# kije/gpu_raytracer

Measured on AMD Instinct MI355X. Metric: Mrays/s, higher is better.
Workload: dtype f32

## Files before the change

### gpu_raytracer_amd/csrc/device_common.h

```cpp
#ifndef RT_DEVICE_COMMON_H
#define RT_DEVICE_COMMON_H

#include <hip/hip_runtime.h>
#include <stdint.h>

#include "device_layout.h"

namespace rtdev {

#define RT_MIN_RAY_DISTANCE 0.00001f
#define RT_F32_MAX 3.402823466e+38f
#define RT_PI 3.14159265358979323846f
#define WAVE 64


struct V3 {
    float x, y, z;
};
__device__ __forceinline__ V3 v3(float x, float y, float z) { return V3{x, y, z}; }
__device__ __forceinline__ V3 ld3(const float* p) { return V3{p[0], p[1], p[2]}; }
__device__ __forceinline__ V3 operator+(V3 a, V3 b) { return v3(a.x + b.x, a.y + b.y, a.z + b.z); }
__device__ __forceinline__ V3 operator-(V3 a, V3 b) { return v3(a.x - b.x, a.y - b.y, a.z - b.z); }
__device__ __forceinline__ V3 operator*(V3 a, V3 b) { return v3(a.x * b.x, a.y * b.y, a.z * b.z); }
__device__ __forceinline__ V3 operator*(V3 a, float s) { return v3(a.x * s, a.y * s, a.z * s); }
// ... 128 lines not shown
}
__device__ __forceinline__ uint32_t ray_octant(const FilterRay& f) {
    return (f.inv.x < 0.0f ? 1u : 0u) | (f.inv.y < 0.0f ? 2u : 0u) | (f.inv.z < 0.0f ? 4u : 0u);
}
__device__ __forceinline__ uint32_t first_slot(uint32_t m, uint32_t oct) {
    uint32_t p = m & 0xFFu;
    if (oct & 1u) p = ((p & 0x55u) << 1) | ((p >> 1) & 0x55u);
    if (oct & 2u) p = ((p & 0x33u) << 2) | ((p >> 2) & 0x33u);
    if (oct & 4u) p = ((p & 0x0Fu) << 4) | (p >> 4);
    return ((uint32_t)__ffs((int)p) - 1u) ^ oct;
}

typedef float f32x2 __attribute__((ext_vector_type(2)));

template <bool COUNT>
__device__ __forceinline__ uint32_t visit_node8(const uint4* __restrict__ nodes, uint32_t idx, const FilterRay& fr, float closest_t, Counts& cnt,
                                                uint32_t& child_base, uint32_t& tri_base, uint32_t& imask, uint32_t& lmask) {
    const uint4* n = nodes + (size_t)idx * 5;
    const uint4 w0 = n[0], w1 = n[1], w2 = n[2], w3 = n[3], w4 = n[4];
    uint32_t w1x = w1.x, w1y = w1.y, w1z = w1.z;
    asm volatile("" : "+v"(w1x), "+v"(w1y), "+v"(w1z));
    if (COUNT) cnt.nodes++;
    const float ax = ldexpf(fr.inv.x, (int)(int8_t)(w0.w & 0xFFu)), ay = ldexpf(fr.inv.y, (int)(int8_t)((w0.w >> 8) & 0xFFu)),
                az = ldexpf(fr.inv.z, (int)(int8_t)((w0.w >> 16) & 0xFFu));
    const float dox = __uint_as_float(w0.x) - fr.o.x, doy = __uint_as_float(w0.y) - fr.o.y, doz = __uint_as_float(w0.z) - fr.o.z;
    const float bx = dox * fr.inv.x, by = doy * fr.inv.y, bz = doz * fr.inv.z;
    const float ex = fmaf(255.0f, fabsf(ax), fabsf(bx)) * RT_FILTER_SLACK;
    const float ey = fmaf(255.0f, fabsf(ay), fabsf(by)) * RT_FILTER_SLACK;
    const float ez = fmaf(255.0f, fabsf(az), fabsf(bz)) * RT_FILTER_SLACK;
    const f32x2 pm = {-1.0f, 1.0f};
    const f32x2 bx2 = __builtin_elementwise_fma((f32x2){ex, ex}, pm, (f32x2){bx, bx});
    const f32x2 by2 = __builtin_elementwise_fma((f32x2){ey, ey}, pm, (f32x2){by, by});
    const f32x2 bz2 = __builtin_elementwise_fma((f32x2){ez, ez}, pm, (f32x2){bz, bz});
    const f32x2 ax2 = {ax, ax}, ay2 = {ay, ay}, az2 = {az, az};
    const bool px = fr.inv.x >= 0.0f, py = fr.inv.y >= 0.0f, pz = fr.inv.z >= 0.0f;
    const uint32_t nxw[2] = {px ? w2.x : w3.z, px ? w2.y : w3.w}, fxw[2] = {px ? w3.z : w2.x, px ? w3.w : w2.y};
    const uint32_t nyw[2] = {py ? w2.z : w4.x, py ? w2.w : w4.y}, fyw[2] = {py ? w4.x : w2.z, py ? w4.y : w2.w};
    const uint32_t nzw[2] = {pz ? w3.x : w4.z, pz ? w3.y : w4.w}, fzw[2] = {pz ? w4.z : w3.x, pz ? w4.w : w3.y};
    const float limit = closest_t * 1.0000153f;
    uint32_t miss = 0;
#pragma unroll
    for (int h = 1; h >= 0; h--) {
#pragma unroll
        for (int i = 3; i >= 0; i--) {
            const f32x2 qx = {(float)((nxw[h] >> (8 * i)) & 0xFFu), (float)((fxw[h] >> (8 * i)) & 0xFFu)};
            const f32x2 qy = {(float)((nyw[h] >> (8 * i)) & 0xFFu), (float)((fyw[h] >> (8 * i)) & 0xFFu)};
            const f32x2 qz = {(float)((nzw[h] >> (8 * i)) & 0xFFu), (float)((fzw[h] >> (8 * i)) & 0xFFu)};
            const f32x2 tx = __builtin_elementwise_fma(qx, ax2, bx2);
            const f32x2 ty = __builtin_elementwise_fma(qy, ay2, by2);
            const f32x2 tz = __builtin_elementwise_fma(qz, az2, bz2);
            const float tmin = fmaxf(fmaxf(tx.x, ty.x), fmaxf(tz.x, 0.0f));
            const float tmax = fminf(fminf(tx.y, ty.y), fminf(tz.y, limit));
            miss = __builtin_amdgcn_alignbit(miss, __float_as_uint(tmax - tmin), 31);
        }
    }
    child_base = w1x;
    tri_base = w1y;
    lmask = w1z & 0xFFu;
    imask = w0.w >> 24;
    return ~miss & (imask | lmask);
}

template <bool COUNT, bool ANY_HIT>
__device__ __forceinline__ void traverse(const DevScene& sc, V3 o, V3 d, uint2* __restrict__ stack, Hit& hit, Counts& cnt, float tmin) {
    if (sc.n_nodes == 0) return;
    const FilterRay fr = make_filter_ray(o, d);
    const uint32_t oct = ray_octant(fr);
    const uint4* __restrict__ nodes = reinterpret_cast<const uint4*>(sc.nodes);
    uint32_t g_base = 0, g_bits = 1u | (1u << 8);
    int sp = 0;
    for (;;) {
        if ((g_bits & 0xFFu) == 0u) {
            if (sp == 0) break;
            sp--;
            const uint2 e = stack[sp * WAVE];
            g_base = e.x;
            g_bits = e.y;
        }
        const uint32_t i = first_slot(g_bits, oct);
        g_bits ^= 1u << i;
        const uint32_t node = g_base + (uint32_t)__popc(__builtin_amdgcn_ubfe(g_bits, 8u, i));
        if (g_bits & 0xFFu) {
            stack[sp * WAVE] = make_uint2(g_base, g_bits);
            sp++;
        }
        uint32_t cb, tb, im, lm;
        const uint32_t hm = visit_node8<COUNT>(nodes, node, fr, hit.t, cnt, cb, tb, im, lm);
        uint32_t t = hm & lm;
        while (t) {
            const uint32_t sl = first_slot(t, oct);
            t ^= 1u << sl;
            const uint32_t first = tb + RT_DEV_LEAF_STRIDE * (uint32_t)__popc(lm & ((1u << sl) - 1u));
            if (test_leaf<COUNT, ANY_HIT>(sc.tris, RT_DEV_LEAF_FLAG | first, o, d, hit, cnt, tmin)) return;
        }
        g_base = cb;
        g_bits = (hm & im) | (im << 8);
    }
}

template <bool COUNT>
__device__ __forceinline__ Hit find_closest(const DevScene& sc, V3 o, V3 d, uint2* stack, Counts& cnt) {
    Hit hit;
    hit.t = RT_F32_MAX;
    hit.prim = RT_PRIM_MISS;
    hit.slot = 0;
    test_spheres(sc, o, d, hit, RT_MIN_RAY_DISTANCE);
    traverse<COUNT, false>(sc, o, d, stack, hit, cnt, RT_MIN_RAY_DISTANCE);
    return hit;
}

template <bool COUNT>
__device__ __forceinline__ bool occluded(const DevScene& sc, V3 o, V3 d, float tmin, float tmax, uint2* stack, Counts& cnt) {
    Hit h;
    h.t = tmax;
    h.prim = RT_PRIM_MISS;
    h.slot = 0;
    test_spheres(sc, o, d, h, tmin);
    if (h.prim != RT_PRIM_MISS) return true;
    traverse<COUNT, true>(sc, o, d, stack, h, cnt, tmin);
    return h.prim != RT_PRIM_MISS;
}

__device__ __forceinline__ V3 evaluate_brdf(const DevMaterial& m, float intensity) {
    V3 albedo = ld3(m.albedo);
    V3 diffuse = albedo / RT_PI;
    float is_metallic = (m.metallic > 0.5f) ? 1.0f : 0.0f;
    V3 metallic_contrib = albedo * intensity * 0.5f;
    V3 dielectric_contrib = diffuse * intensity;
    return metallic_contrib * is_metallic + dielectric_contrib * (1.0f - is_metallic);
}

__device__ __forceinline__ V3 light_contribution(const DevLight& L, const DevMaterial& m, V3 point, V3 normal, V3& to_light_dir,
                                                 float& to_light_dist) {
    V3 dir_light_dir = ld3(L.neg_ndir);
    float dir_intensity = fmaxf(dot(normal, dir_light_dir), 0.0f) * L.intensity;
    V3 to_light = ld3(L.position) - point;
    float distance = length(to_light);
    V3 pld = normalize(to_light);
    float att = f16_round_trip(1.0f / (1.0f + distance * distance * 0.01f));
    float point_intensity = fmaxf(dot(normal, pld), 0.0f) * L.intensity * att;
    float spot_factor = fmaxf(dot(dir_light_dir, pld), 0.0f);
    float spot_intensity = point_intensity * spot_factor;
    float is_dir = (L.light_type == 0) ? 1.0f : 0.0f;
    float is_point = (L.light_type == 1) ? 1.0f : 0.0f;
    float is_spot = (L.light_type == 2) ? 1.0f : 0.0f;
    float final_i = dir_intensity * is_dir + point_intensity * is_point + spot_intensity * is_spot;
    V3 brdf = evaluate_brdf(m, final_i);
    float valid = (final_i > 0.0f) ? 1.0f : 0.0f;
    to_light_dir = (L.light_type == 0) ? dir_light_dir : pld;
    to_light_dist = (L.light_type == 0) ? RT_F32_MAX : distance;
    return brdf * ld3(L.color) * valid;
}

__device__ __forceinline__ V3 calculate_lighting(const DevScene& sc, const DevMaterial& m, V3 point, V3 normal) {
    V3 total = v3(0.0f, 0.0f, 0.0f);
    total = total + ld3(m.albedo) * 0.1f;
    for (uint32_t li = 0; li < sc.n_lights; li++) {
        V3 sd;
        float st;
        total = total + light_contribution(sc.lights[li], m, point, normal, sd, st);
    }
    return total + ld3(m.emission);
}

__device__ __forceinline__ void surface_at(const DevScene& sc, bool sphere, uint32_t slot, V3 point, V3& normal, uint32_t& material_id) {
    if (sphere) {
        const DevSphere& s = sc.spheres[slot];
        normal = normalize(point - ld3(s.center));
        material_id = s.material_id;
    } else {
        const float4* p = reinterpret_cast<const float4*>(sc.tris + slot);
        float4 q0 = p[0], q1 = p[1], q2 = p[2];
        asm volatile("" : "+v"(q0.w), "+v"(q1.x), "+v"(q1.y), "+v"(q1.z), "+v"(q1.w), "+v"(q2.x), "+v"(q2.y));
        V3 e1 = v3(q0.w, q1.x, q1.y);
        V3 e2 = v3(q1.z, q1.w, q2.x);
        normal = normalize(cross(e1, e2));
        material_id = __float_as_uint(q2.y);
    }
}
__device__ __forceinline__ void hit_geometry(const DevScene& sc, const Hit& hit, V3 o, V3 d, V3& point, V3& normal, uint32_t& material_id) {
    point = o + d * hit.t;
    surface_at(sc, (hit.prim & RT_PRIM_SPHERE_FLAG) != 0, hit.slot, point, normal, material_id);
}

__device__ __forceinline__ V3 transmission_mix(const DevMaterial& m, V3 lighting, float tf) {
    float disp_r = ((m.ior + -0.018f) - 1.0f) / (m.ior - 1.0f);
    float disp_g = ((m.ior + 0.0f) - 1.0f) / (m.ior - 1.0f);
    float disp_b = ((m.ior + 0.035f) - 1.0f) / (m.ior - 1.0f);
    float keep = 1.0f - tf;
    return v3(lighting.x * keep + (0.2f * disp_r) * tf, lighting.y * keep + (0.2f * disp_g) * tf,
              lighting.z * keep + (0.3f * disp_b) * tf);
}

__device__ __forceinline__ V3 shade_hit(const DevScene& sc, const Hit& hit, V3 o, V3 d) {
    V3 point, normal;
    uint32_t material_id;
    hit_geometry(sc, hit, o, d, point, normal, material_id);
    if (material_id >= sc.n_materials) return v3(1.0f, 0.0f, 1.0f);
    const DevMaterial m = sc.materials[material_id];
    V3 lighting = calculate_lighting(sc, m, point, normal);
    float tf = fminf(fmaxf(m.transmission, 0.0f), 1.0f);
    if (tf > 0.0f) return transmission_mix(m, lighting, tf);
    return lighting;
}

__device__ __forceinline__ uint32_t unorm8(float v) {
    if (!(v > 0.0f)) return 0u;
    if (v >= 1.0f) return 255u;
    return (uint32_t)floorf(v * 255.0f + 0.5f);
}

struct PixelCoord {
    uint32_t x, y;
    bool valid;
};
__device__ __forceinline__ PixelCoord block_pixel_at(const DevFrame& fr, uint32_t block, uint32_t lane) {
    uint32_t ox, oy, tw, th, blk;
    const uint32_t bpt_x = (fr.tile_size + 7u) >> 3;
    if (fr.single_tile) {
        ox = fr.tile_off_x; oy = fr.tile_off_y; tw = fr.tile_w; th = fr.tile_h;
        blk = block;
    } else {
        const uint32_t bpt = bpt_x * bpt_x;
        uint32_t k = block / bpt;
        blk = block - k * bpt;
        uint32_t tile = fr.tile_first + k * fr.tile_stride;
        uint32_t ty = tile / fr.tiles_x, tx = tile - ty * fr.tiles_x;
        ox = tx * fr.tile_size; oy = ty * fr.tile_size;
        tw = min(fr.tile_size, fr.width - ox);
        th = min(fr.tile_size, fr.height - oy);
    }
    uint32_t by = blk / bpt_x, bx = blk - by * bpt_x;
    uint32_t idx = bx * 8u + (lane & 7u), idy = by * 8u + (lane >> 3);
    PixelCoord pc;
    pc.x = ox + idx;
    pc.y = oy + idy;
    pc.valid = idx < tw && idy < th && pc.x < fr.width && pc.y < fr.height;
    return pc;
}
__device__ __forceinline__ PixelCoord block_pixel(const DevFrame& fr) { return block_pixel_at(fr, blockIdx.x, threadIdx.x); }

struct SimpleRng {
    uint32_t seed;
    __device__ __forceinline__ uint32_t next_u32() {
        seed = seed * 1664525u + 1013904223u;
        return seed;
    }
    __device__ __forceinline__ float next_f32() { return (float)(next_u32() >> 8) / 16777216.0f; }
};

__device__ __forceinline__ SimpleRng rng_for(uint32_t pixel_seed, uint32_t sample) {
    uint32_t h = pixel_seed + sample * 0x9E3779B9u;
    h ^= h >> 16;
    h *= 0x7FEB352Du;
    h ^= h >> 15;
    h *= 0x846CA68Bu;
    h ^= h >> 16;
    return SimpleRng{h};
}

__device__ __forceinline__ V3 run_sum_start(const DevFrame& fr, const DevTargets& tg, size_t pix) {
    if (!tg.run_sum || fr.sample_base == 0) return v3(0.0f, 0.0f, 0.0f);
    const float4 a = reinterpret_cast<const float4*>(tg.run_sum)[pix];
    return v3(a.x, a.y, a.z);
}
__device__ __forceinline__ void run_sum_keep(const DevTargets& tg, size_t pix, V3 sum) {
    if (tg.run_sum) reinterpret_cast<float4*>(tg.run_sum)[pix] = make_float4(sum.x, sum.y, sum.z, 0.0f);
}

__device__ __forceinline__ void sincos_2pi(float u, float& s_out, float& c_out) {
    float f4 = u * 4.0f;
    float qf = floorf(f4);
    int q = (int)qf;
    float x = (f4 - qf) * 1.57079632679489661923f;
    float x2 = x * x;
    float sp = __builtin_fmaf(x2, -2.50521083854417187751e-8f, 2.75573192239858906526e-6f);
    sp = __builtin_fmaf(x2, sp, -1.98412698412698412698e-4f);
    sp = __builtin_fmaf(x2, sp, 8.33333333333333333333e-3f);
    sp = __builtin_fmaf(x2, sp, -1.66666666666666666667e-1f);
    sp = __builtin_fmaf(x2, sp, 1.0f);
    float sn = x * sp;
    float cp = __builtin_fmaf(x2, 2.08767569878680989792e-9f, -2.75573192239858906526e-7f);
    cp = __builtin_fmaf(x2, cp, 2.48015873015873015873e-5f);
    cp = __builtin_fmaf(x2, cp, -1.38888888888888888889e-3f);
    cp = __builtin_fmaf(x2, cp, 4.16666666666666666667e-2f);
    cp = __builtin_fmaf(x2, cp, -0.5f);
    float cs = __builtin_fmaf(x2, cp, 1.0f);
    switch (q & 3) {
        case 0: s_out = sn; c_out = cs; break;
        case 1: s_out = cs; c_out = -sn; break;
        case 2: s_out = -sn; c_out = -cs; break;
        default: s_out = -cs; c_out = sn; break;
    }
}

__device__ __forceinline__ V3 unit_vector(float u1, float u2) {
    float z = 1.0f - 2.0f * u1;
    float r = sqrtf(fmaxf(0.0f, 1.0f - z * z));
    float sn, cs;
    sincos_2pi(u2, sn, cs);
    return v3(r * cs, r * sn, z);
}

#define EXT_EPS 0.001f

struct SegCounts {
// ... 36 lines not shown
```

### gpu_raytracer_amd/csrc/wavefront.hip

```cpp
#include "wavefront.h"
#include <cstdlib>

#include <algorithm>

#include "device_common.h"

using namespace rtdev;

#ifndef RT_WF_REFILL
#define RT_WF_REFILL 16
#endif
#ifndef RT_WF_CHUNK
#define RT_WF_CHUNK 256
#endif
#ifndef RT_WF_ADAPTIVE_CHUNK
#define RT_WF_ADAPTIVE_CHUNK 1
#endif
#ifndef RT_WF_WINDOW
#define RT_WF_WINDOW 512
#endif
#ifndef RT_WF_BLOCK_MAJOR
#define RT_WF_BLOCK_MAJOR 1
#endif
#ifndef RT_WF_SHADE_WAVES
// ... 746 lines not shown
    return GRID_PENDING;
}
template <bool COUNT>
__device__ __forceinline__ uint32_t grid_walk_on(const DevShadowGrid& g, GridPending& pend, uint32_t trips, uint32_t& n_tests, uint32_t& n_entries) {
    const uint4* __restrict__ ovf = g.overflow;
    for (uint32_t k = 0; k < trips; k++) {
        const size_t at = 3 * (size_t)pend.at;
        uint4 q0 = ovf[at], q1 = ovf[at + 1], q2 = ovf[at + 2];
        RT_KEEP4(q0);
        RT_KEEP4(q1);
        RT_KEEP4(q2);
        if (!(__uint_as_float(q0.x) < pend.limit)) return GRID_VISIBLE;
        if (COUNT) n_entries++, n_tests++;
        float t;
        if (moller_trumbore(v3(__uint_as_float(q0.y), __uint_as_float(q0.z), __uint_as_float(q0.w)), v3(__uint_as_float(q1.x), __uint_as_float(q1.y), __uint_as_float(q1.z)),
                            v3(__uint_as_float(q1.w), __uint_as_float(q2.x), __uint_as_float(q2.y)), pend.o, pend.d, t) &&
            t > RT_MIN_RAY_DISTANCE && t < pend.dist)
            return GRID_OCCLUDED;
        pend.at++;
        pend.i++;
        if (pend.i >= pend.count) return GRID_VISIBLE;
        if (pend.i >= RT_WF_GRID_WALK) return GRID_FORWARD;
    }
    return GRID_PENDING;
}

#ifndef RT_WF_GRID_PASS
#define RT_WF_GRID_PASS 3u
#endif
#define RT_WF_GRID_PARK 128u
#define RT_WF_GRID_PARK_WORDS 11u
template <bool COUNT>
__global__ __launch_bounds__(256, RT_WF_GRID_MIN_WAVES) void k_wf_shadow_grid(DevScene sc, rt::WfBuffers wb, const uint32_t* __restrict__ queue) {
    __shared__ DevLight s_lights[RT_WF_MAX_LIGHTS];
    __shared__ DevShadowGrid s_grids[RT_WF_MAX_LIGHTS];
    __shared__ uint32_t s_fwd[4][128];
    __shared__ uint32_t s_park[4][RT_WF_GRID_PARK_WORDS][RT_WF_GRID_PARK];
    if (wb.totals[rt::WF_TOTAL_ERROR] != 0ull) return;
    const uint32_t lane = threadIdx.x & 63u, wave = threadIdx.x >> 6;
    const unsigned long long below = (1ull << lane) - 1ull;
    uint32_t n_fwd = 0, n_park = 0;
    stage_lights(s_lights, sc);
    {
        const uint32_t words = sc.n_lights * (uint32_t)(sizeof(DevShadowGrid) / 4);
        const uint32_t* __restrict__ src = reinterpret_cast<const uint32_t*>(wb.grids);
        uint32_t* dst = reinterpret_cast<uint32_t*>(s_grids);
        for (uint32_t i = threadIdx.x; i < words; i += blockDim.x) dst[i] = src[i];
        __syncthreads();
    }
    uint32_t n_tests = 0, n_entries = 0, n_answered = 0;
    uint32_t(*park)[RT_WF_GRID_PARK] = s_park[wave];
    auto hand_on = [&](bool forward, uint32_t entry, bool flush) {
        const unsigned long long fm = __ballot(forward);
        if (fm != 0ull) {
            if (forward) s_fwd[wave][n_fwd + (uint32_t)__popcll(fm & below)] = entry;
            n_fwd += (uint32_t)__popcll(fm);
        }
        if (n_fwd >= 64u || (flush && n_fwd)) {
            uint32_t at = 0;
            if (lane == 0) at = atomicAdd(&wb.counters[rt::WF_SHADOW2_COUNT], n_fwd);
            at = __shfl(at, 0, WAVE);
            for (uint32_t k = lane; k < n_fwd; k += WAVE) wb.q_shadow2[at + k] = s_fwd[wave][k];
            n_fwd = 0;
        }
    };
    auto park_push = [&](bool pending, const GridPending& pd, uint32_t entry) {
        const unsigned long long pm = __ballot(pending);
        if (pm == 0ull) return;
        if (pending) {
            const uint32_t s = n_park + (uint32_t)__popcll(pm & below);
            park[0][s] = __float_as_uint(pd.o.x), park[1][s] = __float_as_uint(pd.o.y), park[2][s] = __float_as_uint(pd.o.z);
            park[3][s] = __float_as_uint(pd.d.x), park[4][s] = __float_as_uint(pd.d.y), park[5][s] = __float_as_uint(pd.d.z);
            park[6][s] = __float_as_uint(pd.dist), park[7][s] = __float_as_uint(pd.limit);
            park[8][s] = pd.at, park[9][s] = pd.i | (pd.count << 8), park[10][s] = entry;
        }
        n_park += (uint32_t)__popcll(pm);
    };
    auto walk_parked = [&]() {
        const uint32_t take = min(n_park, 64u), first = n_park - take;
        const bool have = lane < take;
        GridPending pd = {};
        uint32_t entry = 0, outcome = GRID_VISIBLE;
        if (have) {
            const uint32_t s = first + lane;
            pd.o = v3(__uint_as_float(park[0][s]), __uint_as_float(park[1][s]), __uint_as_float(park[2][s]));
            pd.d = v3(__uint_as_float(park[3][s]), __uint_as_float(park[4][s]), __uint_as_float(park[5][s]));
            pd.dist = __uint_as_float(park[6][s]), pd.limit = __uint_as_float(park[7][s]);
            pd.at = park[8][s];
            const uint32_t ic = park[9][s];
            pd.i = ic & 0xFFu, pd.count = ic >> 8;
            entry = park[10][s];
            outcome = grid_walk_on<COUNT>(s_grids[entry >> 27], pd, RT_WF_GRID_PASS, n_tests, n_entries);
            if (outcome == GRID_OCCLUDED) atomicAnd(reinterpret_cast<uint32_t*>(&wb.vtx[2 * (size_t)(entry & RT_WF_ID_MASK) + 1]) + 3, ~(1u << (entry >> 27)));
            if (COUNT && outcome <= GRID_OCCLUDED) n_answered++;
        }
        n_park = first;
        park_push(have && outcome == GRID_PENDING, pd, entry);
        hand_on(have && outcome == GRID_FORWARD, entry, false);
    };
    const uint32_t count = wb.counters[rt::WF_EXT_COUNT];
    const uint32_t stride = gridDim.x * blockDim.x;
    uint32_t id_next = blockIdx.x * blockDim.x + threadIdx.x < count ? queue[blockIdx.x * blockDim.x + threadIdx.x] : WF_SENTINEL;
    for (uint32_t base = blockIdx.x * blockDim.x; base < count; base += stride) {
        const uint32_t id = id_next;
        const uint32_t i_next = base + stride + threadIdx.x;
        id_next = i_next < count ? queue[i_next] : WF_SENTINEL;
        uint32_t want = 0;
        V3 point = v3(0, 0, 0), normal = point;
        if (id != WF_SENTINEL) {
            float4 vp = wb.vtx[2 * (size_t)id], vn = wb.vtx[2 * (size_t)id + 1];
            RT_KEEP4(vp);
            RT_KEEP4(vn);
            point = f4v(vp), normal = f4v(vn);
            if (__float_as_uint(vp.w) != 0xFFFFFFFFu) want = __float_as_uint(vn.w);
        }
        uint32_t occluded = 0;
        for (uint32_t li = 0; li < sc.n_lights; li++) {
            const bool mine = (want >> li) & 1u;
            if (__ballot(mine) == 0ull) continue;
            uint32_t outcome = GRID_VISIBLE;
            GridPending pd = {};
            if (mine) {
                outcome = grid_segment_head<COUNT>(sc, s_lights[li], s_grids[li], point, normal, pd, n_tests, n_entries);
                if (outcome == GRID_OCCLUDED) occluded |= 1u << li;
                if (COUNT && outcome <= GRID_OCCLUDED) n_answered++;
            }
            const uint32_t entry = id | (li << 27);
            park_push(mine && outcome == GRID_PENDING, pd, entry);
            hand_on(mine && outcome == GRID_FORWARD, entry, false);
            while (n_park >= 64u) walk_parked();
        }
        if (occluded != 0u) atomicAnd(reinterpret_cast<uint32_t*>(&wb.vtx[2 * (size_t)id + 1]) + 3, ~occluded);
    }
    while (n_park != 0u) walk_parked();
    hand_on(false, 0u, true);
    if (COUNT) {
        const unsigned long long t = wave_sum(n_tests), a = wave_sum(n_answered), en = wave_sum(n_entries);
        if ((threadIdx.x & 63u) == 0) {
            atomicAdd(&wb.totals[rt::WF_TOTAL_TRI_TESTS], t);
            atomicAdd(&wb.totals[rt::WF_TOTAL_GRID_ANSWERED], a);
            atomicAdd(&wb.totals[rt::WF_TOTAL_GRID_ENTRIES], en);
        }
    }
}

__device__ __forceinline__ void wf_end_path(const rt::WfBuffers& wb, uint32_t id, V3 radiance) {
    wb.sample_rad[id] = make_float4(radiance.x, radiance.y, radiance.z, 0.0f);
}

__global__ __launch_bounds__(256, RT_WF_SHADE_WAVES) void k_wf_shade(DevScene sc, DevFrame fr, rt::WfBuffers wb, const uint32_t* __restrict__ queue) {
    __shared__ DevLight s_lights[RT_WF_MAX_LIGHTS];
    if (wb.totals[rt::WF_TOTAL_ERROR] != 0ull) return;
    stage_lights(s_lights, sc);
    const uint32_t count = wb.counters[rt::WF_EXT_COUNT];
    const bool shadows = (fr.flags & RT_FLAG_NO_SHADOWS) == 0;
    const bool to_grids = shadows && wb.grids != nullptr;
    const uint32_t stride = gridDim.x * blockDim.x;
    OutWindow win = {0u, 0u};
    uint32_t n_shadow = 0;
    const uint32_t window = pick_window((count + stride - 1u) / stride, max(1u, sc.n_lights));
    if (blockIdx.x == 0 && threadIdx.x == 0) wb.counters[rt::WF_SHADOW_WINDOW] = window;
    uint32_t id_next = blockIdx.x * blockDim.x + threadIdx.x < count ? queue[blockIdx.x * blockDim.x + threadIdx.x] : WF_SENTINEL;
    for (uint32_t base = blockIdx.x * blockDim.x; base < count; base += stride) {
        const uint32_t id = id_next;
        const uint32_t i_next = base + stride + threadIdx.x;
        id_next = i_next < count ? queue[i_next] : WF_SENTINEL;
        const bool have = id != WF_SENTINEL;
        bool vertex = false;
        V3 point = v3(0, 0, 0), normal = point;
        uint32_t material_id = 0;
        DevMaterial m = {};
        if (have) {
            uint4 h = wb.hit[id];
            asm volatile("" : "+v"(h.x), "+v"(h.y), "+v"(h.z), "+v"(h.w));
            if (h.w == RT_PRIM_MISS) {
                const V3 radiance = f4v(wb.rad[id]) + v3(0.1f, 0.2f, 0.3f) * f4v(wb.thr[id]);
                wf_end_path(wb, id, radiance);
            } else {
                point = v3(__uint_as_float(h.x), __uint_as_float(h.y), __uint_as_float(h.z));
                surface_at(sc, (h.w & RT_PRIM_SPHERE_FLAG) != 0, h.w & ~RT_PRIM_SPHERE_FLAG, point, normal, material_id);
                if (material_id >= sc.n_materials) {
                    const V3 radiance = f4v(wb.rad[id]) + v3(1.0f, 0.0f, 1.0f) * f4v(wb.thr[id]);
                    wf_end_path(wb, id, radiance);
                } else {
                    vertex = true;
                    m = load_material(sc, material_id);
                    wb.vtx[2 * (size_t)id] = make_float4(point.x, point.y, point.z, __uint_as_float(material_id));
                    if (!shadows) wb.vtx[2 * (size_t)id + 1] = make_float4(normal.x, normal.y, normal.z, 0.0f);
                }
            }
        }
        if (have && !vertex) wb.vtx[2 * (size_t)id] = make_float4(0.0f, 0.0f, 0.0f, __uint_as_float(0xFFFFFFFFu));
        if (shadows) {
            uint32_t mask = 0;
            if (vertex) {
                for (uint32_t li = 0; li < sc.n_lights; li++) {
                    V3 sdir;
                    float sdist;
                    const V3 contrib = light_contribution(s_lights[li], m, point, normal, sdir, sdist);
                    if (contrib.x != 0.0f || contrib.y != 0.0f || contrib.z != 0.0f) mask |= 1u << li;
                }
            }
            if (vertex) wb.vtx[2 * (size_t)id + 1] = make_float4(normal.x, normal.y, normal.z, __uint_as_float(mask));
            if (to_grids) {
                n_shadow += (uint32_t)__popc(mask);
                continue;
            }
#if RT_WF_SHADOW_LIGHT_MAJOR
            uint32_t total = 0;
            for (uint32_t li = 0; li < sc.n_lights; li++) total += (uint32_t)__popcll(__ballot((mask >> li) & 1u));
            if (total) {
                uint32_t at = window_reserve(wb.q_shadow, &wb.counters[rt::WF_SHADOW_COUNT], win, window, 0u, 0u, total, wb.q_shadow_cap, &wb.totals[rt::WF_TOTAL_ERROR]);
                n_shadow += (uint32_t)__popc(mask);
                const unsigned long long below = (1ull << (threadIdx.x & 63u)) - 1ull;
                for (uint32_t li = 0; at != WF_NO_SLOT && li < sc.n_lights; li++) {
                    const bool want = (mask >> li) & 1u;
                    const unsigned long long b = __ballot(want);
                    if (want) wb.q_shadow[at + (uint32_t)__popcll(b & below)] = id | (li << 27);
                    at += (uint32_t)__popcll(b);
                }
            }
#else
            const uint32_t mine = (uint32_t)__popc(mask);
            const uint32_t incl = wave_incl_scan(mine), total = __shfl(incl, WAVE - 1, WAVE);
            if (total) {
                uint32_t at = window_reserve(wb.q_shadow, &wb.counters[rt::WF_SHADOW_COUNT], win, window, mine, incl, total, wb.q_shadow_cap, &wb.totals[rt::WF_TOTAL_ERROR]);
                n_shadow += mine;
                while (mask && at != WF_NO_SLOT) {
                    const uint32_t li = (uint32_t)__ffs((int)mask) - 1u;
                    mask &= mask - 1u;
                    wb.q_shadow[at++] = id | (li << 27);
                }
            }
#endif
        }
    }
    window_close(wb.q_shadow, win);
    const unsigned long long ns = wave_sum(n_shadow);
    if ((threadIdx.x & 63u) == 0 && ns) atomicAdd(&wb.totals[rt::WF_TOTAL_SHADOW], ns);
}

__global__ void k_wf_advance(rt::WfBuffers wb) {
    if (threadIdx.x != 0 || blockIdx.x != 0) return;
    uint32_t* c = wb.counters;
    c[rt::WF_EXT_COUNT] = c[rt::WF_EXT_NEXT];
    c[rt::WF_EXT_WINDOW] = c[rt::WF_EXT_WINDOW_NEXT];
    c[rt::WF_EXT_NEXT] = 0;
    c[rt::WF_SHADOW_COUNT] = 0;
    c[rt::WF_SHADOW2_COUNT] = 0;
    c[rt::WF_SHADOW2_CURSOR] = 0;
    c[rt::WF_EXT_CURSOR] = 0;
    c[rt::WF_SHADOW_CURSOR] = 0;
}

__global__ __launch_bounds__(256, RT_WF_SHADE_WAVES) void k_wf_finish(DevScene sc, DevFrame fr, rt::WfBuffers wb, const uint32_t* __restrict__ queue,
                                                  uint32_t* __restrict__ next_queue) {
    __shared__ DevLight s_lights[RT_WF_MAX_LIGHTS];
    if (wb.totals[rt::WF_TOTAL_ERROR] != 0ull) return;
    stage_lights(s_lights, sc);
    const uint32_t count = wb.counters[rt::WF_EXT_COUNT];
    const bool shadows = (fr.flags & RT_FLAG_NO_SHADOWS) == 0;
    const uint32_t stride = gridDim.x * blockDim.x;
    OutWindow win = {0u, 0u};
    uint32_t n_cont = 0;
    const uint32_t window = pick_window((count + stride - 1u) / stride, 1u);
    if (blockIdx.x == 0 && threadIdx.x == 0) wb.counters[rt::WF_EXT_WINDOW_NEXT] = window;
    uint32_t id_next = blockIdx.x * blockDim.x + threadIdx.x < count ? queue[blockIdx.x * blockDim.x + threadIdx.x] : WF_SENTINEL;
    for (uint32_t base = blockIdx.x * blockDim.x; base < count; base += stride) {
        bool cont = false;
        const uint32_t id = id_next;
        const uint32_t i_next = base + stride + threadIdx.x;
        id_next = i_next < count ? queue[i_next] : WF_SENTINEL;
        float4 vp = make_float4(0.0f, 0.0f, 0.0f, __uint_as_float(0xFFFFFFFFu));
        float4 vn = vp, th = vp, ra = vp, rdin = vp;
        if (id != WF_SENTINEL) {
            vp = wb.vtx[2 * (size_t)id];
            vn = wb.vtx[2 * (size_t)id + 1];
            th = wb.thr[id];
            ra = wb.rad[id];
            rdin = wb.ray_d[id];
            RT_KEEP4(vp);
            RT_KEEP4(vn);
            RT_KEEP4(th);
            RT_KEEP4(ra);
            RT_KEEP4(rdin);
        }
        const uint32_t vis = __float_as_uint(vn.w);
        if (__float_as_uint(vp.w) != 0xFFFFFFFFu) {
            const V3 point = f4v(vp), normal = f4v(vn);
            const uint32_t material_id = __float_as_uint(vp.w);
            const DevMaterial m = load_material(sc, material_id);
            V3 throughput = f4v(th), radiance = f4v(ra);
            const uint32_t tw = __float_as_uint(th.w);
            uint32_t channel = tw & 0xFFu;
            const uint32_t depth = tw >> 8;
            SimpleRng rng = {__float_as_uint(ra.w)};
            const bool terminal = depth >= fr.max_bounce;
            V3 lighting = v3(0.0f, 0.0f, 0.0f);
            if (terminal) lighting = lighting + ld3(m.albedo) * 0.1f;
            for (uint32_t li = 0; li < sc.n_lights; li++) {
                V3 sdir;
                float sdist;
                const V3 contrib = light_contribution(s_lights[li], m, point, normal, sdir, sdist);
                const bool nonzero = contrib.x != 0.0f || contrib.y != 0.0f || contrib.z != 0.0f;
                if (nonzero && shadows && !((vis >> li) & 1u)) continue;
                lighting = lighting + contrib;
            }
            lighting = lighting + ld3(m.emission);
            const float tf = fminf(fmaxf(m.transmission, 0.0f), 1.0f);
            if (terminal) {
                V3 out = lighting;
                if (tf > 0.0f) out = transmission_mix(m, lighting, tf);
                radiance = radiance + out * throughput;
                wf_end_path(wb, id, radiance);
            } else {
                radiance = radiance + (lighting * (1.0f - tf)) * throughput;
                const V3 din = f4v(rdin);
                const bool front = dot(normal, din) < 0.0f;
                const V3 nf = front ? normal : -normal;
                bool transmit = false;
                if (tf > 0.0f) transmit = rng.next_f32() < tf;
                V3 ndir, norigin;
                const V3 albedo = ld3(m.albedo);
                bool absorbed = false;
                if (transmit) {
                    if (channel == 3) {
                        uint32_t c = (uint32_t)(rng.next_f32() * 3.0f);
                        channel = c < 2 ? c : 2;
                        throughput = v3(channel == 0 ? throughput.x * 3.0f : 0.0f, channel == 1 ? throughput.y * 3.0f : 0.0f,
                                        channel == 2 ? throughput.z * 3.0f : 0.0f);
                    }
                    const float offs = channel == 0 ? -0.018f : (channel == 1 ? 0.0f : 0.035f);
                    const float ior_c = m.ior + offs;
                    const float eta = front ? (1.0f / ior_c) : ior_c;
                    const float cos_i = -dot(nf, din);
                    const float sin2_t = eta * eta * (1.0f - cos_i * cos_i);
                    if (sin2_t > 1.0f) {
                        ndir = din - nf * (2.0f * dot(din, nf));
                        norigin = point + nf * EXT_EPS;
                    } else {
                        const float cos_t = sqrtf(1.0f - sin2_t);
                        ndir = din * eta + nf * (eta * cos_i - cos_t);
                        norigin = point - nf * EXT_EPS;
                    }
                    ndir = normalize(ndir);
                    throughput = throughput * albedo;
                } else if (m.metallic > 0.5f) {
                    const float u1 = rng.next_f32(), u2 = rng.next_f32();
                    const V3 r = din - nf * (2.0f * dot(din, nf));
                    ndir = normalize(r + unit_vector(u1, u2) * m.roughness);
                    absorbed = !(dot(ndir, nf) > 0.0f);
                    norigin = point + nf * EXT_EPS;
                    if (!absorbed) throughput = throughput * albedo;
                } else {
                    const float u1 = rng.next_f32(), u2 = rng.next_f32();
                    V3 w = nf + unit_vector(u1, u2);
                    if (dot(w, w) < 1e-12f) w = nf;
                    ndir = normalize(w);
                    norigin = point + nf * EXT_EPS;
                    throughput = throughput * albedo;
                }
                if (!absorbed && depth >= 2) {
                    const float p = fminf(fmaxf(fmaxf(fmaxf(throughput.x, throughput.y), throughput.z), 0.05f), 1.0f);
                    if (rng.next_f32() > p) absorbed = true;
                    else throughput = v3(throughput.x / p, throughput.y / p, throughput.z / p);
                }
                if (absorbed) {
                    wf_end_path(wb, id, radiance);
                } else {
                    cont = true;
                    wb.ray_o[id] = make_float4(norigin.x, norigin.y, norigin.z, 0.0f);
                    wb.ray_d[id] = make_float4(ndir.x, ndir.y, ndir.z, 0.0f);
                    wb.thr[id] = make_float4(throughput.x, throughput.y, throughput.z, __uint_as_float(channel | ((depth + 1u) << 8)));
                    wb.rad[id] = make_float4(radiance.x, radiance.y, radiance.z, __uint_as_float(rng.seed));
                }
            }
        }
        const uint32_t mine = cont ? 1u : 0u;
        const uint32_t incl = wave_incl_scan(mine), total = __shfl(incl, WAVE - 1, WAVE);
        if (total) {
            const uint32_t at = window_reserve(next_queue, &wb.counters[rt::WF_EXT_NEXT], win, window, mine, incl, total, wb.q_ext_cap, &wb.totals[rt::WF_TOTAL_ERROR]);
            if (cont && at != WF_NO_SLOT) next_queue[at] = id;
            n_cont += mine;
        }
    }
    window_close(next_queue, win);
    const unsigned long long nc = wave_sum(n_cont);
    if ((threadIdx.x & 63u) == 0 && nc) atomicAdd(&wb.totals[rt::WF_TOTAL_CONTINUATION], nc);
}

__global__ __launch_bounds__(WAVE) void k_wf_resolve(DevFrame fr, rt::WfBuffers wb, DevTargets tg, uint32_t n_samples, uint32_t first_batch,
                                                     uint32_t last_batch) {
    const uint32_t lane = threadIdx.x, b = blockIdx.x;
    const uint32_t q = b * WAVE + lane;
    V3 sum;
    if (!first_batch) sum = f4v(wb.accum[q]);
    else if (tg.run_sum && fr.sample_base) {
        const PixelCoord px = block_pixel_at(fr, b, lane);
        sum = px.valid ? run_sum_start(fr, tg, (size_t)px.y * fr.width + px.x) : v3(0.0f, 0.0f, 0.0f);
    } else sum = v3(0.0f, 0.0f, 0.0f);
    for (uint32_t k = 0; k < n_samples; k++) sum = sum + f4v(wb.sample_rad[(size_t)(RT_WF_BLOCK_MAJOR ? b * n_samples + k : k * wb.n_blocks + b) * WAVE + lane]);
    wb.accum[q] = make_float4(sum.x, sum.y, sum.z, 0.0f);
    if (!last_batch) return;
    const PixelCoord px = block_pixel_at(fr, b, lane);
    if (!px.valid) return;
    const size_t pix = (size_t)px.y * fr.width + px.x;
    run_sum_keep(tg, pix, sum);
    const float n = (float)fr.n_total;
    const V3 color = v3(sum.x / n, sum.y / n, sum.z / n);
    if (tg.rgba32f) reinterpret_cast<float4*>(tg.rgba32f)[pix] = make_float4(color.x, color.y, color.z, 1.0f);
    if (tg.chan[0]) reinterpret_cast<uint32_t*>(tg.chan[0])[pix] = unorm8(color.x) | 0xFF000000u;
    if (tg.chan[1]) reinterpret_cast<uint32_t*>(tg.chan[1])[pix] = (unorm8(color.y) << 8) | 0xFF000000u;
    if (tg.chan[2]) reinterpret_cast<uint32_t*>(tg.chan[2])[pix] = (unorm8(color.z) << 16) | 0xFF000000u;
}

int g_cu_count = 0;
int cu_count() {
    if (g_cu_count == 0) {
        int dev = 0;
        hipDeviceProp_t prop;
        if (hipGetDevice(&dev) == hipSuccess && hipGetDeviceProperties(&prop, dev) == hipSuccess) g_cu_count = prop.multiProcessorCount;
        if (g_cu_count <= 0) g_cu_count = 256;
    }
    return g_cu_count;
}

}

namespace rt {

#ifndef RT_WF_SHADE_BLOCKS_PER_CU
#define RT_WF_SHADE_BLOCKS_PER_CU 16
#endif
uint32_t wf_shading_blocks() {
    static const int per_cu = [] {
        const char* e = std::getenv("RT_WF_SHADE_BLOCKS_PER_CU");
        const int v = e ? std::atoi(e) : 0;
        return v > 0 && v <= 64 ? v : RT_WF_SHADE_BLOCKS_PER_CU;
    }();
    return (uint32_t)(cu_count() * per_cu);
}
size_t wf_queue_slots_for(size_t max_entries, uint32_t per_lane, size_t waves) {
    return max_entries * 4 + (waves + 1) * 2 * ((size_t)wf_min_window(per_lane) + 64u * per_lane) + RT_WF_WINDOW_MAX;
}
size_t wf_queue_slots(size_t max_entries, uint32_t per_lane) { return wf_queue_slots_for(max_entries, per_lane, (size_t)wf_shading_blocks() * 4); }
uint32_t wf_pick_window(uint32_t iters, uint32_t per_lane) { return pick_window(iters, per_lane); }
uint32_t wf_persistent_waves() { return (uint32_t)(cu_count() * RT_WF_WAVES_PER_CU); }
static uint32_t trace_waves_per_cu(uint32_t path_slots) {
    static const int forced = [] { const char* e = std::getenv("RT_WF_WAVES_PER_CU"); const int v = e ? std::atoi(e) : 0; return v > 0 && v <= RT_WF_WAVES_PER_CU ? v : 0; }();
    if (forced) return (uint32_t)forced;
    return path_slots >= (24u << 20) ? (uint32_t)RT_WF_WAVES_PER_CU : RT_WF_WAVES_SMALL;
}

hipError_t wf_beams(const DevScene& sc, const DevFrame& fr, const WfBuffers& wb, hipStream_t s) {
    if (!wb.beam_count || wb.n_blocks == 0) return hipSuccess;
    const hipError_t e = hipMemsetAsync(wb.beam_count + wb.n_blocks, 0, sizeof(uint32_t), s);
    if (e != hipSuccess) return e;
    hipLaunchKernelGGL(k_wf_beams, dim3(wb.n_blocks), dim3(WAVE), 0, s, sc, fr, wb);
    return hipGetLastError();
// ... 58 lines not shown
```

Measured before the change: 3003.

## Add fast light-evaluation path for well-bounded lights and vertices in shade/finish

Adds a specialised light evaluation used when the light and vertex values fall within safe ranges. It computes only the intensity for the light's actual type, chosen wave-uniformly, instead of evaluating all three light models and blending them. A precomputed BRDF factor scales the result, and the code falls back to the full light_contribution when values are out of range or degenerate. In the finish kernel it skips lights the shadow mask marks as occluded, skipping the whole wave when none of its lanes see the light, and redoes the original loop if a negative-zero result could change bit-exactness. This adds more code, branching and register pressure in exchange for less ALU work per light.

```diff
diff --git a/gpu_raytracer_amd/csrc/device_common.h b/gpu_raytracer_amd/csrc/device_common.h
--- a/gpu_raytracer_amd/csrc/device_common.h
+++ b/gpu_raytracer_amd/csrc/device_common.h
@@ -304,6 +304,62 @@
     return brdf * ld3(L.color) * valid;
 }
 
+__device__ __forceinline__ bool light_tame(const DevLight& L) {
+    bool ok = fabsf(L.intensity) <= 0x1p24f, ndir_small = true, ndir_nan = false;
+    for (int c = 0; c < 3; c++) {
+        ok = ok && fabsf(L.position[c]) <= 0x1p40f && fabsf(L.color[c]) <= 0x1p24f;
+        ndir_small = ndir_small && fabsf(L.neg_ndir[c]) <= 2.0f;
+        ndir_nan = ndir_nan || L.neg_ndir[c] != L.neg_ndir[c];
+    }
+    return ok && (ndir_small || ndir_nan);
+}
+
+__device__ __forceinline__ bool vertex_tame(const DevMaterial& m, V3 point, V3 normal) {
+    return fabsf(point.x) <= 0x1p40f && fabsf(point.y) <= 0x1p40f && fabsf(point.z) <= 0x1p40f && fabsf(normal.x) <= 2.0f &&
+           fabsf(normal.y) <= 2.0f && fabsf(normal.z) <= 2.0f && fabsf(m.albedo[0]) <= 0x1p24f && fabsf(m.albedo[1]) <= 0x1p24f &&
+           fabsf(m.albedo[2]) <= 0x1p24f;
+}
+
+struct BrdfFactors {
+    V3 k;
+    float s;
+};
+__device__ __forceinline__ BrdfFactors brdf_factors(const DevMaterial& m) {
+    const bool metal = m.metallic > 0.5f;
+    const V3 albedo = ld3(m.albedo);
+    return BrdfFactors{metal ? albedo : albedo / RT_PI, metal ? 0.5f : 1.0f};
+}
+
+__device__ __forceinline__ bool tame_intensity(const DevLight& L, uint32_t type, V3 point, V3 normal, float& final_i) {
+    const V3 to_light = ld3(L.position) - point;
+    if (type == 0) {
+        final_i = fmaxf(dot(normal, ld3(L.neg_ndir)), 0.0f) * L.intensity;
+        return fmaxf(fmaxf(fabsf(to_light.x), fabsf(to_light.y)), fabsf(to_light.z)) >= 0x1p-49f;
+    }
+    const float distance = length(to_light);
+    const V3 pld = normalize(to_light);
+    const float att = f16_round_trip(1.0f / (1.0f + distance * distance * 0.01f));
+    float i = fmaxf(dot(normal, pld), 0.0f) * L.intensity * att;
+    if (type == 2) i = i * fmaxf(dot(ld3(L.neg_ndir), pld), 0.0f);
+    final_i = type <= 2u ? i : 0.0f;
+    return distance >= 0x1p-50f;
+}
+
+__device__ __forceinline__ bool is_neg0(V3 v) {
+    return __float_as_uint(v.x) == 0x80000000u || __float_as_uint(v.y) == 0x80000000u || __float_as_uint(v.z) == 0x80000000u;
+}
+
+__device__ __forceinline__ V3 tame_contribution(const DevLight& L, const BrdfFactors& b, float final_i) {
+    return ((b.k * final_i) * b.s) * ld3(L.color);
+}
+
+__device__ __forceinline__ uint32_t tame_lights(const DevLight* lights, uint32_t n_lights) {
+    uint32_t bits = 0;
+    for (uint32_t li = 0; li < n_lights; li++)
+        if (light_tame(lights[li])) bits |= 1u << li;
+    return __builtin_amdgcn_readfirstlane(bits);
+}
+
 __device__ __forceinline__ V3 calculate_lighting(const DevScene& sc, const DevMaterial& m, V3 point, V3 normal) {
     V3 total = v3(0.0f, 0.0f, 0.0f);
     total = total + ld3(m.albedo) * 0.1f;
diff --git a/gpu_raytracer_amd/csrc/wavefront.hip b/gpu_raytracer_amd/csrc/wavefront.hip
--- a/gpu_raytracer_amd/csrc/wavefront.hip
+++ b/gpu_raytracer_amd/csrc/wavefront.hip
@@ -922,6 +922,7 @@
     __shared__ DevLight s_lights[RT_WF_MAX_LIGHTS];
     if (wb.totals[rt::WF_TOTAL_ERROR] != 0ull) return;
     stage_lights(s_lights, sc);
+    const uint32_t tame = tame_lights(s_lights, sc.n_lights);
     const uint32_t count = wb.counters[rt::WF_EXT_COUNT];
     const bool shadows = (fr.flags & RT_FLAG_NO_SHADOWS) == 0;
     const bool to_grids = shadows && wb.grids != nullptr;
@@ -964,11 +965,26 @@
         if (shadows) {
             uint32_t mask = 0;
             if (vertex) {
+                const bool fast = vertex_tame(m, point, normal);
+                const BrdfFactors bf = brdf_factors(m);
                 for (uint32_t li = 0; li < sc.n_lights; li++) {
-                    V3 sdir;
-                    float sdist;
-                    const V3 contrib = light_contribution(s_lights[li], m, point, normal, sdir, sdist);
-                    if (contrib.x != 0.0f || contrib.y != 0.0f || contrib.z != 0.0f) mask |= 1u << li;
+                    const DevLight& L = s_lights[li];
+                    float fi = 0.0f;
+                    bool done = false, nonzero = false;
+                    if (fast && ((tame >> li) & 1u)) {
+                        done = tame_intensity(L, __builtin_amdgcn_readfirstlane(L.light_type), point, normal, fi);
+                        if (fi > 0.0f) {
+                            const V3 c = tame_contribution(L, bf, fi);
+                            nonzero = c.x != 0.0f || c.y != 0.0f || c.z != 0.0f;
+                        }
+                    }
+                    if (!done) {
+                        V3 sdir;
+                        float sdist;
+                        const V3 contrib = light_contribution(L, m, point, normal, sdir, sdist);
+                        nonzero = contrib.x != 0.0f || contrib.y != 0.0f || contrib.z != 0.0f;
+                    }
+                    if (nonzero) mask |= 1u << li;
                 }
             }
             if (vertex) wb.vtx[2 * (size_t)id + 1] = make_float4(normal.x, normal.y, normal.z, __uint_as_float(mask));
@@ -1028,6 +1044,7 @@
     __shared__ DevLight s_lights[RT_WF_MAX_LIGHTS];
     if (wb.totals[rt::WF_TOTAL_ERROR] != 0ull) return;
     stage_lights(s_lights, sc);
+    const uint32_t tame = tame_lights(s_lights, sc.n_lights);
     const uint32_t count = wb.counters[rt::WF_EXT_COUNT];
     const bool shadows = (fr.flags & RT_FLAG_NO_SHADOWS) == 0;
     const uint32_t stride = gridDim.x * blockDim.x;
@@ -1066,15 +1083,47 @@
             const uint32_t depth = tw >> 8;
             SimpleRng rng = {__float_as_uint(ra.w)};
             const bool terminal = depth >= fr.max_bounce;
-            V3 lighting = v3(0.0f, 0.0f, 0.0f);
-            if (terminal) lighting = lighting + ld3(m.albedo) * 0.1f;
-            for (uint32_t li = 0; li < sc.n_lights; li++) {
-                V3 sdir;
-                float sdist;
-                const V3 contrib = light_contribution(s_lights[li], m, point, normal, sdir, sdist);
-                const bool nonzero = contrib.x != 0.0f || contrib.y != 0.0f || contrib.z != 0.0f;
-                if (nonzero && shadows && !((vis >> li) & 1u)) continue;
-                lighting = lighting + contrib;
+            const V3 lighting0 = terminal ? v3(0.0f, 0.0f, 0.0f) + ld3(m.albedo) * 0.1f : v3(0.0f, 0.0f, 0.0f);
+            V3 lighting = lighting0;
+            bool walk = shadows;
+            if (walk) {
+                const bool fast = vertex_tame(m, point, normal);
+                const BrdfFactors bf = brdf_factors(m);
+                bool neg0 = is_neg0(lighting);
+                for (uint32_t li = 0; li < sc.n_lights; li++) {
+                    const bool mine = (vis >> li) & 1u;
+                    if (__ballot(mine) == 0ull) continue;
+                    if (!mine) continue;
+                    const DevLight& L = s_lights[li];
+                    float fi = 0.0f;
+                    bool done = false;
+                    V3 contrib = v3(0.0f, 0.0f, 0.0f);
+                    if (fast && ((tame >> li) & 1u)) {
+                        done = tame_intensity(L, __builtin_amdgcn_readfirstlane(L.light_type), point, normal, fi);
+                        if (fi > 0.0f) contrib = tame_contribution(L, bf, fi);
+                    }
+                    if (!done) {
+                        V3 sdir;
+                        float sdist;
+                        contrib = light_contribution(L, m, point, normal, sdir, sdist);
+                    }
+                    lighting = lighting + contrib;
+                    neg0 = neg0 || is_neg0(lighting);
+                }
+                if (neg0) {
+                    walk = false;
+                    lighting = lighting0;
+                }
+            }
+            if (!walk) {
+                for (uint32_t li = 0; li < sc.n_lights; li++) {
+                    V3 sdir;
+                    float sdist;
+                    const V3 contrib = light_contribution(s_lights[li], m, point, normal, sdir, sdist);
+                    const bool nonzero = contrib.x != 0.0f || contrib.y != 0.0f || contrib.z != 0.0f;
+                    if (nonzero && shadows && !((vis >> li) & 1u)) continue;
+                    lighting = lighting + contrib;
+                }
             }
             lighting = lighting + ld3(m.emission);
             const float tf = fminf(fmaxf(m.transmission, 0.0f), 1.0f);
```

New measurement: 3006, median of 5. No clear change (+0.1%).
